# MaciejKozarzewski/AlphaGomoku

Measured on AMD Instinct MI355X. Metric: MCTS simulations/sec (self-play, 15x15 freestyle), higher is better.
Workload: dtype f16 (network, fp32 accumulate) + int/fp32 (tree)

## Files before the change

alphagomoku_amd/csrc/dev_mcts.hpp:

```cpp
#ifndef AGX_DEV_MCTS_HPP_
#define AGX_DEV_MCTS_HPP_

#include "dev_solver.hpp"
#include "root_noise.hpp"
#include "symmetry.hpp"

namespace agx
{
	namespace dev
	{
		__device__ __forceinline__ DNode* nodes_of(const EngineDev &E, int g, int arena) { return E.nodes + E.games[g].node_off[arena]; }
		__device__ __forceinline__ DEdge* edges_of(const EngineDev &E, int g, int arena) { return E.edges + E.games[g].edge_off[arena]; }
		__device__ __forceinline__ int* ht_of(const EngineDev &E, int g) { return E.ht + E.games[g].ht_off; }
		__device__ __forceinline__ void use_game_arenas(EngineDev &E, int g)
		{
			E.node_cap = E.games[g].node_cap;
			E.edge_cap = E.games[g].edge_cap;
			E.ht_cap = E.games[g].ht_cap;
		}

		__device__ inline int cache_seek(const EngineDev &E, const DNode *nodes, const int *ht, u64 hash, const u64 *cboard, int sign, int lane)
		{
			const int mask = E.ht_cap - 1;
			int slot = static_cast<int>(hash & static_cast<u64>(mask));
			for (int probes = 0; probes < E.ht_cap; probes++)
			{
				const int idx = ht[slot];
				if (idx == 0)
					return -1;
				const DNode &nd = nodes[idx - 1];
				bool same = (nd.hash == hash) && (nd.sign_to_move == sign);
				if (same)
				{
					const bool word_ok = (lane < BWORDS) ? (nd.cboard[lane] == cboard[lane]) : true;
					same = (__ballot(!word_ok) == 0);
				}
				if (same)
					return idx - 1;
				slot = (slot + 1) & mask;
			}
			return -1;
		}
		__device__ __forceinline__ void node_head(DNode &dst, const DNode &src)
		{
			dst.edge_begin = src.edge_begin;
			dst.win = src.win;
			dst.draw = src.draw;
			dst.moves_left = src.moves_left;
			dst.visits = src.visits;
			dst.score = src.score;
			dst.n_edges = src.n_edges;
			dst.depth = src.depth;
			dst.vl = src.vl;
			dst.sign_to_move = src.sign_to_move;
			dst.flags = src.flags;
			dst.hash = src.hash;
		}
		__device__ inline int cache_seek_head(const EngineDev &E, const DNode *nodes, const int *ht, u64 hash, const u64 *cboard, int sign, int lane, DNode &head)
		{
			const int mask = E.ht_cap - 1;
			int slot = static_cast<int>(hash & static_cast<u64>(mask));
			for (int probes = 0; probes < E.ht_cap; probes++)
			{
				const int idx = ht[slot];
				if (idx == 0)
					return -1;
				const DNode &nd = nodes[idx - 1];
				DNode h;
				node_head(h, nd);
				const u64 word = (lane < BWORDS) ? nd.cboard[lane] : 0ull;
				bool same = (h.hash == hash) && (h.sign_to_move == sign);
				if (same)
				{
					const bool word_ok = (lane < BWORDS) ? (word == cboard[lane]) : true;
					same = (__ballot(!word_ok) == 0);
				}
				if (same)
				{
					head = h;
					return idx - 1;
				}
				slot = (slot + 1) & mask;
			}
			return -1;
		}
		__device__ inline void cache_insert(const EngineDev &E, int *ht, u64 hash, int node)
		{
			const int mask = E.ht_cap - 1;
			int slot = static_cast<int>(hash & static_cast<u64>(mask));
			while (ht[slot] != 0)
				slot = (slot + 1) & mask;
			ht[slot] = node + 1;
		}

		__device__ inline bool has_leak(const EngineDev &E, const DEdge &e, bool node_found, uint32_t node_score, float node_win, float node_draw)
		{
			if (!node_found || E.leak_threshold >= 1.0f)
				return false;
			if (e.score != s_invert_up(node_score))
				return true;
			const float inv_win = 1.0f - (node_win + node_draw);
			const float dw = e.win - inv_win, dd = e.draw - node_draw;
			return (fabsf(dw) + fabsf(dd)) > E.leak_threshold;
		}

		__device__ __forceinline__ unsigned long long symmetry_mix(unsigned long long z)
		{
			z += 0x9E3779B97F4A7C15ull;
			z = (z ^ (z >> 30)) * 0xBF58476D1CE4E5B9ull;
			z = (z ^ (z >> 27)) * 0x94D049BB133111EBull;
			return z ^ (z >> 31);
		}

		__device__ __forceinline__ void wave_argmax(float &value, int &index)
		{
			const uint32_t bits = __float_as_uint(value);
			const uint32_t key = (bits & 0x80000000u) ? ~bits : (bits | 0x80000000u);
			const uint32_t best = wave_reduce_umax(key);
			const uint32_t mine = (key == best) ? (0x7FFFFFFFu - static_cast<uint32_t>(index)) : 0u;
			index = static_cast<int>(0x7FFFFFFFu - wave_reduce_umax(mine));
			value = __uint_as_float((best & 0x80000000u) ? (best & 0x7FFFFFFFu) : ~best);
		}
		__device__ __forceinline__ uint32_t wave_max_u32(uint32_t v)
		{
			return wave_reduce_umax(v);
		}

		__device__ inline int select_edge(const EngineDev &E, const DNode &nd, const DEdge *edges, int lane, unsigned long long &edge_reads, const float *noisy_priors)
		{
			const int total = nd.visits + nd.vl;
			float c_puct = E.c_puct;
			if (E.c_scale != 0.0f)
				c_puct = static_cast<float>(static_cast<double>(E.c_puct) + static_cast<double>(E.c_scale) * det_log(static_cast<double>(total)));
			const float parent_sqrt_visit = static_cast<float>(static_cast<double>(c_puct) * sqrt(static_cast<double>(total)));
			float initial_q = 0.0f;
			if (E.init_to == 1)
				initial_q = nd.win + 0.5f * nd.draw;
			else if (E.init_to == 2)
				initial_q = 0.5f;

			float best_value = -3.402823466e+38f;
			int best = 0x7FFFFFFF;
			for (int i = lane; i < nd.n_edges; i += 64)
			{
				const DEdge e = edges[nd.edge_begin + i];
				float value;
				switch (s_pv(e.score))
				{
					case 0:
						value = -1000.0f + s_distance(e.score);
						break;
					case 1:
						value = 0.5f;
						break;
					case 3:
						value = +1000.0f - s_distance(e.score);
						break;
					default:
					{
						const int vl = e.flag_vl & 0x7FFF;
						const bool being_expanded = (e.flag_vl & 0x8000u) != 0;
						const float visits = 1.0e-8f + e.visits;
						const float virtual_loss = static_cast<float>(vl);
						const float vl_factor = visits / (visits + virtual_loss);
						const float expectation = e.win + 0.5f * e.draw;
						float Q;
						if (E.init_to == 0)
							Q = being_expanded ? -1000.0f : expectation * vl_factor;
						else
						{
							Q = initial_q;
							if (being_expanded)
								Q = -1000.0f;
							else if (e.visits > 0)
								Q = expectation * vl_factor;
						}
						const float prior = (noisy_priors != nullptr) ? noisy_priors[i] : e.prior;
						const float U = prior * parent_sqrt_visit / (1.0f + e.visits + vl);
						value = Q + U;
						break;
					}
				}
				if (value > best_value)
				{
					best_value = value;
					best = i;
				}
			}
			edge_reads += nd.n_edges;
			wave_argmax(best_value, best);
			return nd.edge_begin + best;
		}

		__device__ inline void correct_information_leak(DNode *nodes, DEdge *edges, const DTask &t, int path_len, int final_node, int lane)
		{
			float child_win = nodes[final_node].win, child_draw = nodes[final_node].draw;
			uint32_t child_score = nodes[final_node].score;
			for (int i = path_len - 1; i >= 0; i--)
			{
				const int node = t.path_node[i], e = t.path_edge[i];
				DNode nd;
				node_head(nd, nodes[node]);
				DEdge ed = edges[e];
				const float cw = ed.win, cd = ed.draw;
				const float tw = 1.0f - (child_win + child_draw), td = child_draw;
				const float scale = static_cast<float>(ed.visits) / static_cast<float>(nd.visits);
				const float nw = nd.win + (tw - cw) * scale, ndr = nd.draw + (td - cd) * scale;
				ed.win = tw;
				ed.draw = td;
				nd.win = nw;
				nd.draw = ndr;
				const uint32_t new_score = s_invert_up(child_score);
				ed.score = static_cast<uint16_t>(new_score);
				uint32_t result = 0;
				for (int j = lane; j < nd.n_edges; j += 64)
					result = max(result, (nd.edge_begin + j == e) ? new_score : static_cast<uint32_t>(edges[nd.edge_begin + j].score));
				result = wave_max_u32(result);
				if (((nd.flags & 4) != 0) || s_win(result) || s_unproven(result))
					nd.score = static_cast<uint16_t>(result);
				if (lane == 0)
				{
					nodes[node].win = nd.win;
					nodes[node].draw = nd.draw;
					nodes[node].score = nd.score;
					edges[e].win = ed.win;
					edges[e].draw = ed.draw;
					edges[e].score = ed.score;
				}
				child_win = nd.win;
				child_draw = nd.draw;
				child_score = nd.score;
			}
		}
		__device__ inline void cancel_virtual_loss(DNode *nodes, DEdge *edges, const DTask &t, int path_len, int lane)
		{
			for (int i = lane; i < path_len; i += 64)
			{
				nodes[t.path_node[i]].vl--;
				DEdge &e = edges[t.path_edge[i]];
				e.flag_vl = static_cast<uint16_t>((e.flag_vl & 0x8000u) | (((e.flag_vl & 0x7FFF) - 1) & 0x7FFF));
			}
		}

		__device__ inline u64 full_hash(const EngineDev &E, const uint8_t *board, int sign, int lane)
		{
			u64 h = 0;
			for (int i = lane; i < E.hw; i += 64)
				h ^= E.nc_keys[3 + 3 * i + board[i]];
			return wave_reduce_xor64(h) ^ E.nc_keys[sign];
		}
	}
}

#endif
```

alphagomoku_amd/csrc/engine.hip:

```cpp
#include "agx_internal.hpp"
#include "engine_types.hpp"
#include "dev_mcts.hpp"
#include "tables_host.hpp"
#include "renju_static.hpp"
#include "root_noise.hpp"
#include "sample_v201.hpp"

#include <vector>
#include <thread>
#include <chrono>
#include <mutex>
#include <cstring>
#include <algorithm>

using namespace agx;
using namespace agx::dev;

namespace
{
	__device__ __forceinline__ void select_batch(EngineDev &E, int tg, int g, int lane, uint8_t *sh_board, u64 *sh_cboard, const u64 *sh_keys)
	{
		GameState &gs = E.games[tg];
		GameState &ls = E.games[g];
		DNode *nodes = nodes_of(E, tg, gs.arena);
		DEdge *edges = edges_of(E, tg, gs.arena);
		const int *ht = ht_of(E, tg);
		const int n = E.n;

		int n_tasks = ls.n_tasks;
		int trials = 2 * E.batch_limit;
		unsigned long long st_levels = 0, st_edges = 0, st_leaks = 0, st_proven = 0, st_dup = 0;
		while (n_tasks < E.batch_limit)
		{
			const int root = gs.root;
			const int sims = (root < 0) ? 0 : nodes[root].visits;
			if (sims > E.max_sims)
				break;
			if (E.noise_type != 0 && root >= 0 && !gs.noise_ready && nodes[root].n_edges > 0)
			{
				if (lane == 0)
				{
					const DNode rn = nodes[root];
					const DEdge *root_edges = edges + rn.edge_begin;
					make_root_noise(E.noise_type, E.noise_weight, E.noise_seed, gs.opening_id, gs.n_moves, rn.n_edges, [&](int i) { return root_edges[i].prior; },
							E.noise + static_cast<size_t>(tg) * E.hw);
					gs.noise_ready = 1;
				}
				__threadfence_block();
				__syncthreads();
			}
			DTask &t = E.tasks[static_cast<size_t>(g) * E.batch + n_tasks];
			n_tasks++;
			for (int i = lane; i < E.hw; i += 64)
				sh_board[i] = gs.board[i];
			if (lane < BWORDS)
				sh_cboard[lane] = gs.cboard[lane];
			__syncthreads();
			int path_len = 0, final_node = -1, out = 0, sign = gs.sign_to_move;
			u64 hash = gs.root_hash;
			int last_edge = -1;
			int node = root;
			DNode nd;
			if (node >= 0)
				node_head(nd, nodes[node]);
			while (node >= 0)
			{
				if (path_len >= PATH_CAP)
				{
					if (lane == 0)
						ls.error = ERR_PATH_CAPACITY;
					break;
				}
				const int e = select_edge(E, nd, edges, lane, st_edges, (node == root && gs.noise_ready) ? E.noise + static_cast<size_t>(tg) * E.hw : nullptr);
				st_levels++;
				const DEdge ee = edges[e];
				const uint32_t mv = ee.move;
				const int s = mv & 3, cell = ((mv >> 2) & 127) * n + ((mv >> 9) & 127);
				const uint16_t flag_vl = static_cast<uint16_t>((ee.flag_vl & 0x8000u) | (((ee.flag_vl & 0x7FFF) + 1) & 0x7FFF));
				if (lane == 0)
				{
					sh_board[cell] = static_cast<uint8_t>(s);
					sh_cboard[cell >> 5] |= static_cast<u64>(s) << (2 * (cell & 31));
					t.path_node[path_len] = node;
					t.path_edge[path_len] = e;
					nodes[node].vl = static_cast<int16_t>(nd.vl + 1);
					edges[e].flag_vl = flag_vl;
				}
				hash ^= sh_keys[3 + 3 * cell] ^ sh_keys[3 + 3 * cell + s] ^ sh_keys[sign] ^ sh_keys[3 - s];
				sign = 3 - s;
				path_len++;
				last_edge = e;
				__syncthreads();
				if (s_proven(ee.score))
				{
					out = 2;
					break;
				}
				DNode child;
				node = cache_seek_head(E, nodes, ht, hash, sh_cboard, sign, lane, child);
				final_node = node;
				if (node < 0 && lane == 0)
					edges[e].flag_vl = static_cast<uint16_t>(flag_vl | 0x8000u);
				if (has_leak(E, ee, node >= 0, child.score, child.win, child.draw))
				{
					out = 1;
					break;
				}
				nd = child;
			}
			for (int i = lane; i < E.hw; i += 64)
				t.board[i] = sh_board[i];
			if (lane < BWORDS)
				t.cboard[lane] = sh_cboard[lane];
			if (lane == 0)
			{
				t.path_len = path_len;
				t.final_node = final_node;
				t.n_edges = 0;
				t.flags = t.flags & (TF_STATICALLY_SOLVED | TF_RECURSIVELY_SOLVED);
				t.sign_to_move = sign;
				t.score = s_unknown(0);
				t.win = 0.0f;
				t.draw = 0.0f;
				t.needs_nn = 0;
				t.hash = hash;
				if (out == 0 && path_len > gs.max_depth)
					gs.max_depth = path_len;
			}
			__syncthreads();
			if (path_len == 0)
				break;
			for (int i = 0; i < n_tasks - 1; i++)
			{
				const DTask &o = E.tasks[static_cast<size_t>(g) * E.batch + i];
				if (o.path_len > 0 && o.path_edge[o.path_len - 1] == last_edge)
				{
					st_dup++;
					break;
				}
			}
			if (out == 1)
			{
				correct_information_leak(nodes, edges, t, path_len, final_node, lane);
				cancel_virtual_loss(nodes, edges, t, path_len, lane);
				st_leaks++;
				n_tasks--;
			}
			if (out == 2 && lane == 0)
			{
				const uint32_t sc = edges[last_edge].score;
				float w, d;
				s_to_value(sc, w, d);
				t.final_node = -1;
				t.sign_to_move = 3 - sign;
				t.score = sc;
				t.win = w;
				t.draw = d;
				t.flags |= TF_BY_SOLVER | TF_SKIP_EDGE_GENERATION;
			}
			if (out == 2)
				st_proven++;
			__syncthreads();
			if (--trials <= 0)
				break;
		}
		if (lane == 0)
		{
			ls.n_tasks = n_tasks;
			ls.stats[2] += st_leaks;
			ls.stats[3] += st_proven;
			ls.stats[6] += st_levels;
			ls.stats[7] += st_edges;
			ls.stats[9] += st_dup;
		}
	}
	__global__ __launch_bounds__(64) void k_select(EngineDev E)
	{
		__shared__ uint8_t sh_board[MAXHW];
		__shared__ u64 sh_cboard[BWORDS];
		__shared__ u64 sh_keys[3 * (1 + MAXHW)];
		const int g = E.g0 + blockIdx.x, lane = threadIdx.x;
		const int tg = E.shared_tree ? 0 : g;
		GameState &gs = E.games[tg];
		if (!gs.active || gs.error != 0 || gs.outcome != 0 || gs.grow_pending)
			return;
		use_game_arenas(E, tg);
		for (int i = lane; i < 3 * (1 + E.hw); i += 64)
			sh_keys[i] = E.nc_keys[i];
		if (!E.shared_tree)
		{
			if (!gs.solve_pending)
				select_batch(E, g, g, lane, sh_board, sh_cboard, sh_keys);
			return;
		}
		for (int t = E.grp_first; t < E.grp_first + E.grp_count; t++)
		{
			if (E.games[t].error == 0)
				select_batch(E, 0, t, lane, sh_board, sh_cboard, sh_keys);
			__syncthreads();
		}
	}

	constexpr float SPEC_PARK_FRACTION = 0.90f;
	struct ParkCtl
	{
			int count;
			int threshold;
	};
	template<class SH>
	__device__ __forceinline__ void park_copy_tails(const SH &sh, const EngineDev &E, int from, int to, int lane)
	{
		lane = fresh_lane(lane);
// ... 1113 lines not shown
						const int src = (r < K) ? (0xFFFF - static_cast<int>(sort_keys[r] & 0xFFFFu)) : 0;
						g_mv[c] = e_move[src];
						g_sc[c] = e_score[src];
						g_p[c] = e_prior[src];
						g_w[c] = e_win[src];
						g_d[c] = e_draw[src];
						kept += __popcll(__ballot(r < K && g_p[c] >= threshold));
					}
					__syncthreads();
#pragma unroll
					for (int c = 0; c < 7; c++)
					{
						const int r = c * 64 + lane;
						if (r < kept)
						{
							e_move[r] = g_mv[c];
							e_score[r] = g_sc[c];
							e_prior[r] = g_p[c];
							e_win[r] = g_w[c];
							e_draw[r] = g_d[c];
						}
					}
					__syncthreads();
					n_e = kept;
				}
				float sum = 0.0f;
				for (int base = 0; base < n_e; base += 64)
				{
					const int mine_i = __float_as_int((base + lane < n_e) ? e_prior[base + lane] : 0.0f);
					const int m = min(64, n_e - base);
					int j = 0;
					for (; j + 4 <= m; j += 4)
					{
						sum += __int_as_float(__builtin_amdgcn_readlane(mine_i, j));
						sum += __int_as_float(__builtin_amdgcn_readlane(mine_i, j + 1));
						sum += __int_as_float(__builtin_amdgcn_readlane(mine_i, j + 2));
						sum += __int_as_float(__builtin_amdgcn_readlane(mine_i, j + 3));
					}
					for (; j < m; j++)
						sum += __int_as_float(__builtin_amdgcn_readlane(mine_i, j));
				}
				if (sum == 0.0f)
				{
					const float u = 1.0f / n_e;
					for (int i = lane; i < n_e; i += 64)
						e_prior[i] = u;
				}
				else
				{
					const float inv = 1.0f / sum;
					for (int i = lane; i < n_e; i += 64)
						e_prior[i] = e_prior[i] * inv;
				}
				__syncthreads();
			}
			else
				n_e = 0;

			int final_node = t.final_node;
			if (n_e > 0)
			{
				const int found = cache_seek(E, nodes, ht, t.hash, t.cboard, sign, lane);
				if (found < 0)
				{
					const int nid = gs.n_nodes, ebeg = gs.n_edges;
					if (nid >= E.node_cap || ebeg + n_e > E.edge_cap || 2 * (nid + 1) > E.ht_cap)
					{
						if (lane == 0)
							gs.error = (nid >= E.node_cap) ? ERR_NODE_CAPACITY : ((ebeg + n_e > E.edge_cap) ? ERR_EDGE_CAPACITY : ERR_HASH_TABLE);
						__syncthreads();
						return;
					}
					uint32_t max_score = 0;
					for (int i = lane; i < n_e; i += 64)
					{
						DEdge e;
						e.prior = e_prior[i];
						e.win = e_win[i];
						e.draw = e_draw[i];
						e.visits = 0;
						e.move = e_move[i];
						e.score = e_score[i];
						e.flag_vl = 0;
						e.pad = 0;
						edges[ebeg + i] = e;
						max_score = max(max_score, static_cast<uint32_t>(e_score[i]));
					}
					max_score = wave_max_u32(max_score);
					if (lane < BWORDS)
						nodes[nid].cboard[lane] = t.cboard[lane];
					if (lane == 0)
					{
						DNode &nd = nodes[nid];
						nd.edge_begin = ebeg;
						nd.n_edges = static_cast<int16_t>(n_e);
						nd.depth = static_cast<int16_t>(gs.n_moves + path_len);
						nd.vl = 0;
						nd.sign_to_move = static_cast<uint8_t>(sign);
						nd.pad8 = 0;
						nd.hash = t.hash;
						nd.visits = 1;
						const float tmp = static_cast<float>(1.0 / 1);
						float w = 0.0f + (win - 0.0f) * tmp, d = 0.0f + (draw - 0.0f) * tmp;
						nd.win = fmaxf(0.0f, fminf(1.0f, w));
						nd.draw = fmaxf(0.0f, fminf(1.0f, d));
						nd.moves_left = 0.0f + (moves_left - 0.0f) / 1;
						uint16_t nf = 0;
						if ((flags & TF_MUST_DEFEND) || (n_e + nd.depth) == hw)
							nf |= 4;
						nf |= ((flags & TF_STATICALLY_SOLVED) ? 8 : 0) | ((flags & TF_RECURSIVELY_SOLVED) ? 16 : 0) | ((flags & TF_MUST_DEFEND) ? 32 : 0);
						if (path_len == 0)
							nf |= 2;
						nd.flags = nf;
						nd.score = static_cast<uint16_t>(s_unknown(0));
						if ((nf & 4) || s_win(max_score) || s_unproven(max_score))
							nd.score = static_cast<uint16_t>(max_score);
						cache_insert(E, ht, t.hash, nid);
						gs.n_nodes = nid + 1;
						gs.n_edges = ebeg + n_e;
						if (path_len == 0)
							gs.root = nid;
					}
					final_node = nid;
					__syncthreads();
				}
				else
				{
					final_node = found;
					wasted++;
					if (path_len > 0)
					{
						const DEdge le = edges[t.path_edge[path_len - 1]];
						if (has_leak(E, le, true, nodes[found].score, nodes[found].win, nodes[found].draw))
							correct_information_leak(nodes, edges, t, path_len, final_node, lane);
					}
				}
			}

			if (lane == 0)
			{
				t.final_node = final_node;
				t.win = win;
				t.draw = draw;
				t.moves_left = moves_left;
				t.flags = flags;
			}
			__syncthreads();
		}

		for (int k = 0; k < n_tasks; k++)
		{
			DTask &t = E.tasks[static_cast<size_t>(g) * E.batch + k];
			const float win = t.win, draw = t.draw;
			const int path_len = t.path_len, sign = t.sign_to_move, final_node = t.final_node;
			float ml = t.moves_left;
			bool have_child = final_node >= 0;
			uint32_t child_score = have_child ? nodes[final_node].score : 0u;
#if AGX_WIDE_BACKUP
			if (path_len <= 64)
			{
				const bool mine = lane < path_len;
				const int node = mine ? t.path_node[lane] : 0, e = mine ? t.path_edge[lane] : 0;
				DNode nd;
				node_head(nd, nodes[node]);
				DEdge ed = edges[e];
				float ml_i = ml;
				for (int k = path_len - 1; k > lane; k--)
					ml_i += 1.0f;
				float vw = win, vd = draw;
				if (nd.sign_to_move != sign)
				{
					vw = 1.0f - (win + draw);
					vd = draw;
				}
				nd.visits++;
				const float tn = static_cast<float>(1.0 / nd.visits);
				nd.win = fmaxf(0.0f, fminf(1.0f, nd.win + (vw - nd.win) * tn));
				nd.draw = fmaxf(0.0f, fminf(1.0f, nd.draw + (vd - nd.draw) * tn));
				ed.visits++;
				const float te = 1.0f / ed.visits;
				ed.win = fmaxf(0.0f, fminf(1.0f, ed.win + (vw - ed.win) * te));
				ed.draw = fmaxf(0.0f, fminf(1.0f, ed.draw + (vd - ed.draw) * te));
				nd.moves_left += (ml_i - nd.moves_left) / nd.visits;
				nd.vl--;
				ed.flag_vl = static_cast<uint16_t>(((ed.flag_vl & 0x7FFF) - 1) & 0x7FFF);
				uint32_t others = 0;
				constexpr int LEVELS = 8, LOADS = (MAXHW + 63) / 64;
				for (int base = 0; base < path_len; base += LEVELS)
				{
					uint32_t sc[LEVELS][LOADS];
#pragma unroll
					for (int u = 0; u < LEVELS; u++)
					{
						const int lv = min(base + u, path_len - 1);
						const int eb = __builtin_amdgcn_readlane(nd.edge_begin, __builtin_amdgcn_readfirstlane(lv));
						const int ne = __builtin_amdgcn_readlane(static_cast<int>(nd.n_edges), __builtin_amdgcn_readfirstlane(lv));
						const int ee = __builtin_amdgcn_readlane(e, __builtin_amdgcn_readfirstlane(lv));
#pragma unroll
						for (int jj = 0; jj < LOADS; jj++)
						{
							const int j = lane + 64 * jj;
							sc[u][jj] = (base + u < path_len && j < ne && eb + j != ee) ? static_cast<uint32_t>(edges[eb + j].score) : 0u;
						}
					}
#pragma unroll
					for (int u = 0; u < LEVELS; u++)
					{
						uint32_t m = 0;
#pragma unroll
						for (int jj = 0; jj < LOADS; jj++)
							m = max(m, sc[u][jj]);
						m = wave_max_u32(m);
						if (lane == base + u)
							others = m;
					}
// ... 183 lines not shown
		for (int i = tid; i < E.hw; i += 256)
			h ^= E.nc_keys[3 + 3 * i + gs.board[i]];
		block_reduce_xor(h, scratch, tid);
		if (tid == 0)
			gs.root_hash = h ^ E.nc_keys[gs.sign_to_move];
		__syncthreads();
	}

	template<int TPB, bool DropRoot = false>
	__device__ void rebase_tree(const EngineDev &E0, int t, int tid, u64 *scratch, int *scan_nodes, int *scan_edges)
	{
		EngineDev E = E0;
		use_game_arenas(E, t);
		GameState &gs = E.games[t];
		const int lane = tid & 63, wave = tid >> 6;
		DNode *nodes = nodes_of(E, t, gs.arena);
		DEdge *edges = edges_of(E, t, gs.arena);
		DNode *dst_nodes = nodes_of(E, t, gs.arena ^ 1);
		DEdge *dst_edges = edges_of(E, t, gs.arena ^ 1);
		int *ht = ht_of(E, t);
		for (int i = tid; i < E.ht_cap; i += TPB)
			ht[i] = 0;
		const int total = gs.n_nodes;
		int node_base = 0, edge_base = 0;
		u64 drop_hash = 0;
		if constexpr (DropRoot)
		{
			for (int i = tid; i < E.hw; i += TPB)
				drop_hash ^= E.nc_keys[3 + 3 * i + gs.board[i]];
			block_reduce_xor<TPB>(drop_hash, scratch, tid);
			drop_hash ^= E.nc_keys[gs.sign_to_move];
		}
		__syncthreads();
		for (int base = 0; base < total; base += TPB)
		{
			const int i = base + tid;
			int keep = 0, ne = 0;
			if (i < total)
			{
				keep = 1;
				u64 differs = 0;
				for (int w = 0; w < BWORDS; w++)
				{
					const u64 from = gs.cboard[w], to = nodes[i].cboard[w];
					if (((from ^ to) & from) != 0)
						keep = 0;
					differs |= from ^ to;
				}
				if constexpr (DropRoot)
				{
					if (differs == 0 && nodes[i].hash == drop_hash && nodes[i].sign_to_move == gs.sign_to_move)
						keep = 0;
				}
				ne = keep ? nodes[i].n_edges : 0;
			}
			scan_nodes[tid] = keep;
			scan_edges[tid] = ne;
			__syncthreads();
			for (int o = 1; o < TPB; o <<= 1)
			{
				const int a = (tid >= o) ? scan_nodes[tid - o] : 0, b = (tid >= o) ? scan_edges[tid - o] : 0;
				__syncthreads();
				scan_nodes[tid] += a;
				scan_edges[tid] += b;
				__syncthreads();
			}
			int cp_src = 0, cp_dst = 0;
			if (keep)
			{
				const int ni = node_base + scan_nodes[tid] - 1, eb = edge_base + scan_edges[tid] - ne;
				DNode nd = nodes[i];
				cp_src = nd.edge_begin;
				cp_dst = eb;
				nd.edge_begin = eb;
				dst_nodes[ni] = nd;
				const int mask = E.ht_cap - 1;
				int slot = static_cast<int>(nd.hash & static_cast<u64>(mask));
				while (atomicCAS(&ht[slot], 0, ni + 1) != 0)
					slot = (slot + 1) & mask;
			}
			{
				const u64 *src64 = reinterpret_cast<const u64*>(edges);
				u64 *dst64 = reinterpret_cast<u64*>(dst_edges);
				for (int k = 0; k < 64; k++)
				{
					const int words = 3 * __builtin_amdgcn_readlane(ne, k);
					if (words == 0)
						continue;
					const size_t so = 3 * static_cast<size_t>(__builtin_amdgcn_readlane(cp_src, k)), dof = 3 * static_cast<size_t>(__builtin_amdgcn_readlane(cp_dst, k));
					for (int d = lane; d < words; d += 256)
					{
						const u64 w0 = src64[so + d];
						const u64 w1 = (d + 64 < words) ? src64[so + d + 64] : 0ull;
						const u64 w2 = (d + 128 < words) ? src64[so + d + 128] : 0ull;
						const u64 w3 = (d + 192 < words) ? src64[so + d + 192] : 0ull;
						dst64[dof + d] = w0;
						if (d + 64 < words)
							dst64[dof + d + 64] = w1;
						if (d + 128 < words)
							dst64[dof + d + 128] = w2;
						if (d + 192 < words)
							dst64[dof + d + 192] = w3;
					}
				}
			}
			node_base += scan_nodes[TPB - 1];
			edge_base += scan_edges[TPB - 1];
			__syncthreads();
		}
		u64 h = 0;
		for (int i = tid; i < E.hw; i += TPB)
			h ^= E.nc_keys[3 + 3 * i + gs.board[i]];
		block_reduce_xor<TPB>(h, scratch, tid);
		if (tid == 0)
		{
			gs.root_hash = h ^ E.nc_keys[gs.sign_to_move];
			gs.n_nodes = node_base;
			gs.n_edges = edge_base;
			gs.arena ^= 1;
			gs.generation = (gs.generation + 1) % 64;
			gs.max_depth = 0;
		}
		__syncthreads();
		if (wave == 0)
		{
			const int found = cache_seek(E, dst_nodes, ht, gs.root_hash, gs.cboard, gs.sign_to_move, lane);
			if (lane == 0)
			{
				gs.root = found;
				if (found >= 0)
					dst_nodes[found].flags |= 2;
			}
		}
		__syncthreads();
	}

	__global__ __launch_bounds__(256) void k_begin(EngineDev E)
	{
		__shared__ u64 scratch[4];
		const int g = blockIdx.x, tid = threadIdx.x;
		GameState &gs = E.games[g];
		__shared__ int sh_id;
		if (tid == 0)
		{
			sh_id = E.shared_tree ? 0 : g;
			gs.generation = 0;
			gs.error = 0;
			gs.games_done = 0;
			gs.arena = 0;
			for (int i = 0; i < 12; i++)
				gs.stats[i] = 0;
		}
		__syncthreads();
		if (E.match_mode)
		{
			clear_tree_and_table(E, g, tid);
			if (tid == 0)
			{
				gs.active = 0;
				gs.root = -1;
				gs.n_nodes = 0;
				gs.n_edges = 0;
				gs.n_tasks = 0;
				gs.need_move = 0;
				gs.solve_pos = 0;
				gs.solve_pending = 0;
				park_forget_game(E, g);
				gs.outcome = 0;
				gs.n_moves = 0;
				gs.restart_id = (g < E.n_games / 2) ? -1 : 0;
				gs.match_score[0] = gs.match_score[1] = gs.match_score[2] = gs.match_score[3] = 0;
			}
		}
		else if (sh_id < E.n_openings)
			begin_game(E, g, sh_id, tid, scratch);
		else if (tid == 0)
		{
			gs.active = 0;
			gs.restart_id = -1;
		}
	}

	constexpr int ADV_THREADS = 1024;
	__global__ __launch_bounds__(ADV_THREADS) void k_advance(EngineDev E)
	{
// ... 1887 lines not shown
	cfg->game_end_capacity = 0;
	cfg->speculative_solver = 0;
	cfg->speculative_waves = 0;
	cfg->force_expand_root = 1;
	cfg->search_buffers = 0;
	cfg->noise_type = 0;
	cfg->noise_weight = 0.0f;
	cfg->noise_seed = 0x2545F4914F6CDD1Dull;
	return AGX_OK;
}

#if defined(AGX_QUICK) && !defined(AGX_QUICK_RENJU)
#define AGX_QUICK_RENJU false
#endif
typedef void (*SpecKernel)(EngineDev, int);
static SpecKernel spec_kernel(int rules, int n)
{
#ifdef AGX_QUICK
	(void) rules;
	(void) n;
	return k_search_spec<AGX_QUICK_RENJU, 15>;
#else
	if (rules == AGX_RENJU)
		return (n == 15) ? k_search_spec<true, 15> : k_search_spec<true, 0>;
	if (n == 15)
		return k_search_spec<false, 15>;
	return (n == 20) ? k_search_spec<false, 20> : k_search_spec<false, 0>;
#endif
}
static int spec_resident_waves_per_cu(int rules, int n)
{
	int blocks = 0;
	if (hipOccupancyMaxActiveBlocksPerMultiprocessor(&blocks, reinterpret_cast<const void*>(spec_kernel(rules, n)), 64, 0) != hipSuccess || blocks <= 0)
	{
		(void) hipGetLastError();
		return 12;
	}
	return blocks;
}
static int engine_create(const AgxEngineConfig *cfg, AgxEngine **out, int sizing_cus)
{
	AGX_REQUIRE(cfg != nullptr && out != nullptr, AGX_ERR_INVALID, "agx_engine_create: null argument");
	AGX_REQUIRE(cfg->rules >= 0 && cfg->rules <= AGX_CARO6, AGX_ERR_INVALID, "agx_engine_create: unknown rules %d", cfg->rules);
	AGX_REQUIRE(cfg->board_size >= 5 && cfg->board_size <= MAXN, AGX_ERR_UNSUPPORTED, "agx_engine_create: board size %d not in [5, %d]", cfg->board_size, MAXN);
	AGX_REQUIRE(cfg->n_games > 0 && cfg->max_batch_size > 0 && cfg->max_simulations > 0, AGX_ERR_INVALID, "agx_engine_create: non-positive sizes");
	AGX_REQUIRE(cfg->tss_max_positions >= 1 && cfg->tss_max_positions <= 1000, AGX_ERR_UNSUPPORTED, "agx_engine_create: tss_max_positions must be in [1, 1000]");
	AGX_REQUIRE(cfg->init_to >= 0 && cfg->init_to <= 3, AGX_ERR_INVALID, "agx_engine_create: init_to must be 0..3");
	AGX_REQUIRE(cfg->solver_yield_fraction >= 0.0f && cfg->solver_yield_fraction <= 1.0f, AGX_ERR_INVALID, "agx_engine_create: solver_yield_fraction must be in [0, 1]");
	AGX_REQUIRE(cfg->final_selector >= 0 && cfg->final_selector <= 5, AGX_ERR_INVALID, "agx_engine_create: final_selector must be 0..5");
	AGX_REQUIRE(cfg->noise_type >= 0 && cfg->noise_type <= 3, AGX_ERR_INVALID, "agx_engine_create: noise_type must be 0 (none), 1 (custom), 2 (dirichlet) or 3 (gumbel)");
	AGX_REQUIRE(cfg->policy_temperature >= 0.0f, AGX_ERR_INVALID, "agx_engine_create: policy_temperature must not be negative");
	AGX_REQUIRE(!cfg->match_mode || cfg->n_games % 2 == 0, AGX_ERR_INVALID, "agx_engine_create: match_mode pairs the trees, n_games must be even");
	AGX_REQUIRE(cfg->noise_weight >= 0.0f && cfg->noise_weight <= 1.0f, AGX_ERR_INVALID, "agx_engine_create: noise_weight must be in [0, 1]");
	AGX_REQUIRE(cfg->search_buffers >= 0 && cfg->search_buffers <= 2, AGX_ERR_INVALID, "agx_engine_create: search_buffers must be 0, 1 or 2");
	{
		const int threads = std::max(1, cfg->search_threads), buffers = (cfg->search_buffers == 2) ? 2 : 1;
		AGX_REQUIRE((threads == 1 && buffers == 1) || (threads * buffers == cfg->n_games && !cfg->match_mode && cfg->solver_yield_fraction == 0.0f), AGX_ERR_INVALID,
				"agx_engine_create: search_threads > 1 / search_buffers = 2 make the pool ONE tree searched by n_games task buffers: n_games must equal "
				"search_threads x buffers (%d x %d), no match_mode, no yielding", threads, buffers);
	}
	AGX_REQUIRE(cfg->record_format >= 0 && cfg->record_format <= 3, AGX_ERR_INVALID, "agx_engine_create: record_format must be 0..3 (bit 0 edge snapshots, bit 1 format-201 samples)");

	AgxEngine *e = new AgxEngine();
	e->cfg = *cfg;
	e->sizing_only = sizing_cus > 0;
	e->sizing_cus = sizing_cus;
	if (const char *fuse = std::getenv("AGX_FUSE_SELECT"))
		e->fuse_select = std::atoi(fuse) != 0;
	EngineDev &d = e->dev;
	std::memset(&d, 0, sizeof(d));
	d.rules = cfg->rules;
	d.n = cfg->board_size;
	d.hw = d.n * d.n;
	d.draw_after = (cfg->draw_after > 0) ? cfg->draw_after : d.hw;
	d.n_games = cfg->n_games;
	d.batch = cfg->max_batch_size;
	d.max_sims = cfg->max_simulations;
	d.c_puct = cfg->exploration_constant;
	d.c_scale = cfg->exploration_scaling;
	d.init_to = cfg->init_to;
	d.leak_threshold = cfg->information_leak_threshold;
	d.expansion_threshold = cfg->policy_expansion_threshold;
	d.max_children = (cfg->max_children > 0) ? cfg->max_children : 0x7FFFFFFF;
	d.tss_max_nodes = cfg->tss_max_positions;
	d.tss_max_depth = 100;
	d.solve_time_ticks = 0ull;
	d.batch_limit = d.batch;
	d.yield_fraction = cfg->solver_yield_fraction;
	d.final_selector = cfg->final_selector;
	d.use_symmetries = cfg->use_symmetries;
	d.symmetry_seed = cfg->symmetry_seed;
	d.noise_type = (cfg->noise_weight > 0.0f) ? cfg->noise_type : 0;
	d.noise_weight = cfg->noise_weight;
	d.noise_seed = cfg->noise_seed;
	const size_t buckets = round_pow2(std::max<size_t>(cfg->tss_table_entries, 4)) / 4;
	d.tt_bucket_mask = buckets - 1;
	d.zobrist_seed = cfg->zobrist_seed;
	d.node_cap = cfg->node_capacity > 0 ? cfg->node_capacity : 8192;
	d.edge_cap = cfg->edge_capacity > 0 ? cfg->edge_capacity : 524288;
	d.edge_cap += d.edge_cap & 1;
	d.ht_cap = static_cast<int>(round_pow2(4 * static_cast<size_t>(d.node_cap)));
	d.act_cap = d.hw * (d.hw + 1) / 2 + 64;
	d.record_cap = cfg->record_capacity > 0 ? cfg->record_capacity : d.n_games * d.hw;
	d.record_edge_cap = cfg->record_edge_capacity > 0 ? cfg->record_edge_capacity : d.record_cap * 64;
	d.record_format = cfg->record_format;
	d.sample_cap = cfg->record_sample_capacity > 0 ? cfg->record_sample_capacity
			: static_cast<int>(std::min<size_t>(static_cast<size_t>(d.record_cap) * (16 + 6 * static_cast<size_t>(d.hw) + 2), 0x7FFFFFF0u));
	d.game_end_cap = cfg->game_end_capacity > 0 ? cfg->game_end_capacity : std::max(2 * d.n_games, d.record_cap / 16);

	HostTables tables;
	build_host_tables(cfg->rules, tables);
	std::vector<uint64_t> nc_keys(3 + 3 * d.hw);
	uint64_t st = cfg->zobrist_seed ^ 0x5851F42D4C957F2Dull;
	for (auto &k : nc_keys)
		k = splitmix64(st);
	e->zobrist.resize(4 * d.hw);
	st = cfg->zobrist_seed;
	for (auto &k : e->zobrist)
		k = splitmix64(st);

	int status = AGX_OK;
	const size_t G = d.n_games;
#define AGX_TRY(expr) if (status == AGX_OK) status = (expr)
	AGX_TRY(dev_alloc(e, &d.games, G));
	const double reserve = (cfg->arena_reserve >= 0.0f) ? cfg->arena_reserve : 1.0;
	const size_t node_total = static_cast<size_t>(static_cast<double>(G * 2 * d.node_cap) * (1.0 + reserve));
	const size_t edge_total = static_cast<size_t>(static_cast<double>(G * 2 * d.edge_cap) * (1.0 + reserve));
	const size_t ht_total = static_cast<size_t>(static_cast<double>(G * d.ht_cap) * (1.0 + reserve));
	AGX_TRY(dev_alloc(e, &d.nodes, node_total));
	AGX_TRY(dev_alloc(e, &d.edges, edge_total));
	AGX_TRY(dev_alloc(e, &d.ht, ht_total));
	AGX_TRY(dev_alloc(e, &d.heap, 1));
	AGX_TRY(dev_alloc(e, &d.free_bundles, static_cast<size_t>(ARENA_CLASSES) * G));
	AGX_TRY(dev_alloc(e, &d.tasks, G * d.batch));
	e->speculative = cfg->speculative_solver != 0 && cfg->tss_max_positions <= 250 && cfg->max_batch_size <= 16;
	if (e->speculative)
	{
		int cus = e->sizing_cus, device_of_engine = 0;
		if (!e->sizing_only)
		{
			(void) hipGetDevice(&device_of_engine);
			(void) hipDeviceGetAttribute(&cus, hipDeviceAttributeMultiprocessorCount, device_of_engine);
		}
		const int per_cu = spec_resident_waves_per_cu(cfg->rules, cfg->board_size);
		e->spec_waves = (cfg->speculative_waves > 0) ? cfg->speculative_waves : std::min<long long>(static_cast<long long>(per_cu) * std::max(1, cus), std::max<long long>(64, static_cast<long long>(G) * cfg->max_batch_size));
		e->spec_waves = std::min(e->spec_waves, SPEC_QUEUE_SLACK);
	}
	const bool parking = e->speculative && cfg->rules == AGX_RENJU && cfg->solver_yield_fraction > 0.0f && !cfg->match_mode && std::max(1, cfg->search_threads) == 1;
	const size_t areas = G + static_cast<size_t>(std::max(e->spec_waves, 16)) + (parking ? SPEC_PARK_POOL : 0);
	d.park_area0 = static_cast<int>(G) + std::max(e->spec_waves, 16);
	d.spec_on = e->speculative ? 1 : 0;
	d.park_fraction = parking ? SPEC_PARK_FRACTION : 0.0f;
	if (const char *pf = std::getenv("AGX_PARK_FRACTION"))
		if (parking && std::atof(pf) > 0.0)
			d.park_fraction = std::min(1.0f, static_cast<float>(std::atof(pf)));
	AGX_TRY(dev_alloc(e, &d.park_slot, G * d.batch));
	AGX_TRY(dev_alloc(e, &d.park_owner, SPEC_PARK_POOL));
	AGX_TRY(dev_alloc(e, &d.parts_done, 2 * G));
	if (!e->sizing_only)
		(void) hipMemset(d.parts_done, 0, 2 * G * sizeof(int));
	AGX_TRY(dev_alloc(e, &d.park_lds, parking ? static_cast<size_t>(SPEC_PARK_POOL) * SPEC_PARK_WORDS : 1));
	if (!e->sizing_only)
		(void) hipMemset(d.park_slot, 0, G * d.batch * sizeof(int));
	if (!e->sizing_only)
		(void) hipMemset(d.park_owner, 0, SPEC_PARK_POOL * sizeof(int));
	AGX_TRY(dev_alloc(e, &d.act, areas * d.act_cap));
// ... 2190 lines not shown
```

alphagomoku_amd/csrc/engine_types.hpp:

```cpp
#ifndef AGX_ENGINE_TYPES_HPP_
#define AGX_ENGINE_TYPES_HPP_

#include <cstdint>

namespace agx
{
	constexpr int MAXN = 20;
	constexpr int MAXHW = MAXN * MAXN;
	constexpr int BWORDS = 13;
	constexpr int PATH_CAP = 256;
	constexpr int SPEC_PARK_POOL = 128;
	constexpr int SPEC_PARK_WORDS = 2048 + 8;
	constexpr int MAX_FRAMES = 104;
	constexpr int OPENING_CAP = 32;

	struct alignas(16) FrameBytes { uint32_t w[8]; };

	struct DEdge
	{
			float prior;
			float win;
			float draw;
			int32_t visits;
			uint16_t move;
			uint16_t score;
			uint16_t flag_vl;
			uint16_t pad;
	};
	static_assert(sizeof(DEdge) == 24, "edge record must stay 24 bytes");

	struct DNode
	{
			int32_t edge_begin;
			float win;
			float draw;
			float moves_left;
			int32_t visits;
			uint16_t score;
			int16_t n_edges;
			int16_t depth;
			int16_t vl;
			uint8_t sign_to_move;
			uint8_t pad8;
			uint16_t flags;
			uint64_t hash;
			uint64_t cboard[BWORDS];
	};
	static_assert(sizeof(DNode) == 144, "node record layout");

	enum TaskFlags : uint32_t
	{
		TF_MUST_DEFEND = 1, TF_BY_NETWORK = 2, TF_BY_SOLVER = 4, TF_SKIP_EDGE_GENERATION = 8, TF_STATICALLY_SOLVED = 16, TF_RECURSIVELY_SOLVED = 32
	};

	struct DTask
	{
			int32_t path_len;
			int32_t final_node;
			int32_t n_edges;
			uint32_t flags;
			int32_t sign_to_move;
			uint32_t score;
			float win;
			float draw;
			float moves_left;
			int32_t needs_nn;
			int32_t symmetry;
			int32_t pad;
			uint64_t hash;
			uint64_t cboard[BWORDS];
			int32_t path_node[PATH_CAP];
			int32_t path_edge[PATH_CAP];
			uint8_t board[MAXHW];
			uint16_t emove[MAXHW];
			uint16_t escore[MAXHW];
	};

	struct GameState
	{
			int32_t active;
			int32_t sign_to_move;
			int32_t n_moves;
			int32_t outcome;
			int32_t root;
			int32_t n_nodes;
			int32_t n_edges;
			int32_t arena;
			int32_t n_tasks;
			int32_t need_move;
			int32_t generation;
			int32_t error;
			int32_t opening_id;
			int32_t games_done;
			int32_t solve_pos;
			int32_t solve_pending;
			int32_t nn_queued;
			int32_t noise_ready;
			int32_t my_sign;
			int32_t restart_id;
			int32_t match_score[4];
			int32_t arena_class;
			int32_t grow_pending;
			int32_t node_cap, edge_cap, ht_cap, grow_count;
			int32_t grow_owner, max_depth;
			uint64_t node_off[2], edge_off[2], ht_off;
			uint64_t new_node_off[2], new_edge_off[2], new_ht_off;
			uint64_t root_hash;
			uint64_t cboard[BWORDS];
			unsigned long long prof[8];
			unsigned long long dprof[24];
			unsigned long long spec_stats[4];
			unsigned long long stats[12];
			uint8_t board[MAXHW];
			uint16_t moves[MAXHW];
	};

	struct MoveRecordHeader
	{
			int32_t game_serial;
			int32_t move_number;
			uint16_t move;
			uint16_t root_score;
			int32_t root_visits;
			float root_win;
			float root_draw;
			int32_t n_edges;
			int32_t edge_offset;
			int32_t root_flags;
			int32_t game_slot;
			int32_t game_index;
			int32_t sample_offset;
			int32_t sample_bytes;
			int32_t outcome;
	};
	struct GameEndRecord
	{
			int32_t game_serial, game_slot, game_index;
			int32_t outcome;
			int32_t n_moves;
			uint16_t moves[MAXHW];
	};

	constexpr int SPEC_OV_CAP = 256;
	constexpr int SPEC_COUNTER0 = 64;
	constexpr int SPEC_QUEUE_SLACK = 8192;
	constexpr int N_COUNTERS = 192;
	struct SpecTask
	{
			int32_t solved;
			int32_t count;
			int32_t overflow;
			int32_t nodes;
			uint32_t flags0;
			float moves_left0;
			uint32_t pad[2];
			uint32_t dirty[SPEC_OV_CAP / 32];
			uint32_t keys[SPEC_OV_CAP];
	};

	constexpr int ARENA_CLASSES = 6;

	struct ArenaBundle
	{
			uint64_t node_off[2], edge_off[2], ht_off;
	};
	struct ArenaHeap
	{
			uint64_t node_cursor, edge_cursor, ht_cursor;
			uint64_t node_total, edge_total, ht_total;
			int32_t free_count[ARENA_CLASSES];
			int32_t free_capacity;
			int32_t grows, releases, failures, lock;
	};

	enum EngineError : int32_t
	{
		ERR_NONE = 0, ERR_NODE_CAPACITY = 1, ERR_EDGE_CAPACITY = 2, ERR_PATH_CAPACITY = 3, ERR_ACTION_STACK = 4, ERR_HASH_TABLE = 5, ERR_RECORDS = 6, ERR_FRAMES = 7, ERR_SPEC_STATE = 8,
		ERR_OVERLAY = 100
	};

	struct EngineDev
	{
			int rules, n, hw, draw_after;
			int n_games, batch, max_sims;
			int batch_limit;
			float c_puct, c_scale;
			int init_to;
			float leak_threshold, expansion_threshold;
			int max_children;
			float policy_temperature;
			int tss_max_nodes, tss_max_depth;
			unsigned long long solve_time_ticks;
			unsigned long long zobrist_seed;
			unsigned long long tt_bucket_mask;
			int node_cap, edge_cap, ht_cap, act_cap;
			int record_cap, record_edge_cap;
			int record_format;
			int sample_cap;
			int game_end_cap;
			int n_openings;
			float yield_fraction;
			int yield_counter;
			int final_selector, use_symmetries;
			unsigned long long symmetry_seed;
			int noise_type;
			float noise_weight;
			unsigned long long noise_seed;
			float *noise;
			int g0;
			int nn_counter;
			GameState *games;
			DNode *nodes;
			DEdge *edges;
			int *ht;
			ArenaHeap *heap;
			ArenaBundle *free_bundles;
			DTask *tasks;
			uint32_t *act;
			uint16_t *list_spill;
			FrameBytes *frame_spill;
			uint64_t *snap_spill;
			uint64_t *tt;
			const uint8_t *t_pattern;
			const uint8_t *t_ho3;
			const uint8_t *t_threat;
			const uint8_t *t_threat_packed;
			const uint16_t *t_defense;
			const uint64_t *nc_keys;
			const uint64_t *zob;
			const uint16_t *openings;
			uint32_t *nn_features;
			float *nn_policy;
			float *nn_value;
			float *nn_q;
			int has_q;
			int match_merged;
			int prune_root;
			int match_mode;
			int shared_tree;
			int search_buffers;
			int tt_mod;
			int grp_first, grp_count;
			int spec_on;
			int spec_group;
			int *spec_watchdog;
			unsigned long long *spec_trace;
			unsigned long long *spec_prof;
			int spec_waves;
			int *spec_items;
			int *spec_left;
			SpecTask *spec_tasks;
			uint64_t *spec_overlay;
			int *park_slot;
			int *park_owner;
			int *parts_done;
			uint64_t *park_lds;
			int park_area0;
			float park_fraction;
			int *nn_list;
			int *counters;
			MoveRecordHeader *records;
			DEdge *record_edges;
			uint8_t *samples;
			GameEndRecord *game_ends;
	};
}

#endif
```

include/agx.h:

```cpp
#ifndef AGX_H_
#define AGX_H_

#include <stddef.h>
#include <stdint.h>

#ifdef __cplusplus
extern "C" {
#endif

#define AGX_OK 0
#define AGX_ERR_INVALID 1
#define AGX_ERR_HIP 2
#define AGX_ERR_UNSUPPORTED 3
#define AGX_ERR_STATE 4

enum AgxRules { AGX_FREESTYLE = 0, AGX_STANDARD = 1, AGX_RENJU = 2, AGX_CARO5 = 3, AGX_CARO6 = 4 };

enum AgxSign { AGX_NONE = 0, AGX_CROSS = 1, AGX_CIRCLE = 2, AGX_ILLEGAL = 3 };

const char* agx_last_error(void);
int agx_version(void);
const char* agx_build_hash(void);
int agx_set_device(int device);
int agx_device_count(int* count);
// ... 10 lines not shown
	int action_values;
} AgxNetDesc;

typedef struct AgxNet AgxNet;

size_t agx_net_blob_floats(const AgxNetDesc* desc);
int agx_net_create(const AgxNetDesc* desc, AgxNet** out);
int agx_net_load_weights(AgxNet* net, const float* h_blob, size_t n_floats);
int agx_nn_forward(AgxNet* net, const uint32_t* d_features, int batch, float* d_policy, float* d_value, void* stream);
int agx_nn_forward_pvq(AgxNet* net, const uint32_t* d_features, int batch, float* d_policy, float* d_value, float* d_action_values, void* stream);
int agx_net_description(const AgxNet* net, AgxNetDesc* out);
int agx_net_set_launch_width(AgxNet* net, int workgroups);
int agx_net_destroy(AgxNet* net);

int agx_nn_forward_indirect(AgxNet* net, const uint32_t* d_features, const int* d_slot_list, const int* d_count, int max_batch,
		float* d_policy, float* d_value, void* stream);
int agx_nn_forward_indirect_pvq(AgxNet* net, const uint32_t* d_features, const int* d_slot_list, const int* d_count, int max_batch,
		float* d_policy, float* d_value, float* d_action_values, void* stream);

enum AgxNetArchitecture { AGX_ARCH_RESNET = 0, AGX_ARCH_CONVNEXT = 1, AGX_ARCH_BOTTLENECK = 2 };
size_t agx_net_blob_floats_ex(const AgxNetDesc* desc, int architecture, int moves_left);
int agx_net_create_ex(const AgxNetDesc* desc, int architecture, int moves_left, AgxNet** out);
int agx_net_architecture(const AgxNet* net, int* architecture, int* moves_left);
int agx_nn_forward_pvqm(AgxNet* net, const uint32_t* d_features, int batch, float* d_policy, float* d_value, float* d_action_values,
		float* d_moves_left, void* stream);
int agx_nn_forward_indirect_pvqm(AgxNet* net, const uint32_t* d_features, const int* d_slot_list, const int* d_count, int max_batch,
		float* d_policy, float* d_value, float* d_action_values, float* d_moves_left, void* stream);

typedef struct AgxEngineConfig
{
	int rules;
	int board_size;
	int draw_after;
	int n_games;
	int max_batch_size;
	int max_simulations;
	float exploration_constant;
	float exploration_scaling;
	int init_to;
	float information_leak_threshold;
	float policy_expansion_threshold;
	int tss_max_positions;
	uint64_t tss_table_entries;
	uint64_t zobrist_seed;
	int node_capacity;
	int edge_capacity;
	int record_capacity;
	int record_edge_capacity;
	float solver_yield_fraction;
	int final_selector;
	int use_symmetries;
	uint64_t symmetry_seed;
	int max_children;
	int noise_type;
	float noise_weight;
	uint64_t noise_seed;
	int action_values;
	int match_mode;
	float policy_temperature;
	float arena_reserve;
	int search_threads;
	int record_format;
	int record_sample_capacity;
	int game_end_capacity;
	int speculative_solver;
	int speculative_waves;
	int force_expand_root;
	int search_buffers;
} AgxEngineConfig;

typedef struct AgxEngine AgxEngine;

typedef struct AgxEngineBuffers
{
	uint32_t* d_nn_features;
	float* d_nn_policy;
	float* d_nn_value;
	float* d_nn_action_values;
	int* d_nn_list;
	int* d_nn_count;
	int slots;
	int cells;
} AgxEngineBuffers;

typedef struct AgxEngineStats
{
	unsigned long long evaluated_nodes;
	unsigned long long network_evaluations;
	unsigned long long information_leaks;
	unsigned long long proven_edge_visits;
	unsigned long long wasted_expansions;
	unsigned long long duplicate_selections;
	unsigned long long solver_nodes;
	unsigned long long select_levels;
	unsigned long long select_edge_reads;
	unsigned long long moves_played;
	unsigned long long peak_nodes;
	unsigned long long peak_edges;
	int games_finished;
	int openings_taken;
	int active_games;
	int records_used;
	int record_edges_used;
	int first_error;
	int arena_grows;
	int arena_releases;
	int arena_failures;
	int arena_max_class;
	float arena_heap_used;
	int speculative_parks;
	unsigned long long speculative_solves;
	unsigned long long speculative_reruns;
	unsigned long long speculative_deferrals;
} AgxEngineStats;

typedef struct AgxEdgeView
{
	float prior, win, draw;
	int32_t visits;
	uint16_t move;
	uint16_t score;
	uint16_t flag_and_virtual_loss;
	uint16_t reserved;
} AgxEdgeView;

typedef struct AgxGameInfo
{
	int active, sign_to_move, n_moves, outcome, error, opening_id, games_done, n_nodes, n_edges;
	int root_visits;
	float root_win, root_draw;
	int root_score;
	int root_edges;
	int grow_pending;
	int arena_class;
	float root_moves_left;
	int max_depth;
} AgxGameInfo;

typedef struct AgxMoveRecord
{
	int game_serial, move_number;
	uint16_t move, root_score;
	int root_visits;
	float root_win, root_draw;
	int n_edges, edge_offset;
	int root_flags;
	int game_slot;
	int game_index;
	int sample_offset;
	int sample_bytes;
	int outcome;
} AgxMoveRecord;

typedef struct AgxGameEnd
{
	int game_serial, game_slot, game_index;
	int outcome;
	int n_moves;
	uint16_t moves[400];
} AgxGameEnd;

typedef struct AgxSavedGame
{
	int game_slot, game_index;
	int opening_id, sign_to_move, nn_queued, n_moves;
	uint16_t moves[400];
// ... 360 lines not shown
```

Measured before the change: 1.035 million.

## Cache child node links in edge padding to skip hash-table probes during selection

Reuses the spare 16-bit pad field of each edge as a direct link to the child node index, filled on expansion, cache hit and first lookup. Selection then checks the linked node's hash and sign instead of probing the hash table and comparing the full board. It also broadcasts the chosen edge from the owning lane with readlane instead of re-reading it from memory. Links are cleared when the tree is rebased. The fast path is limited to nodes below 65535, and a mismatched link aborts with a new error code, which is a correctness risk.

```diff
diff --git a/alphagomoku_amd/csrc/dev_mcts.hpp b/alphagomoku_amd/csrc/dev_mcts.hpp
--- a/alphagomoku_amd/csrc/dev_mcts.hpp
+++ b/alphagomoku_amd/csrc/dev_mcts.hpp
@@ -84,6 +84,13 @@
 			}
 			return -1;
 		}
+		__device__ __forceinline__ int linked_seek_head(const DNode *nodes, int n_nodes, uint32_t child, u64 hash, int sign, DNode &head)
+		{
+			if (static_cast<int>(child) > n_nodes)
+				return -2;
+			node_head(head, nodes[child - 1]);
+			return (head.hash == hash && head.sign_to_move == sign) ? static_cast<int>(child) - 1 : -2;
+		}
 		__device__ inline void cache_insert(const EngineDev &E, int *ht, u64 hash, int node)
 		{
 			const int mask = E.ht_cap - 1;
@@ -126,7 +133,8 @@
 			return wave_reduce_umax(v);
 		}
 
-		__device__ inline int select_edge(const EngineDev &E, const DNode &nd, const DEdge *edges, int lane, unsigned long long &edge_reads, const float *noisy_priors)
+		__device__ inline int select_edge(const EngineDev &E, const DNode &nd, const DEdge *edges, int lane, unsigned long long &edge_reads, const float *noisy_priors,
+				DEdge &chosen)
 		{
 			const int total = nd.visits + nd.vl;
 			float c_puct = E.c_puct;
@@ -141,6 +149,7 @@
 
 			float best_value = -3.402823466e+38f;
 			int best = 0x7FFFFFFF;
+			DEdge mine = { };
 			for (int i = lane; i < nd.n_edges; i += 64)
 			{
 				const DEdge e = edges[nd.edge_begin + i];
@@ -185,10 +194,22 @@
 				{
 					best_value = value;
 					best = i;
+					mine = e;
 				}
 			}
 			edge_reads += nd.n_edges;
 			wave_argmax(best_value, best);
+			const int owner = __builtin_amdgcn_readfirstlane(best & 63);
+			chosen.prior = __int_as_float(__builtin_amdgcn_readlane(__float_as_int(mine.prior), owner));
+			chosen.win = __int_as_float(__builtin_amdgcn_readlane(__float_as_int(mine.win), owner));
+			chosen.draw = __int_as_float(__builtin_amdgcn_readlane(__float_as_int(mine.draw), owner));
+			chosen.visits = __builtin_amdgcn_readlane(mine.visits, owner);
+			const uint32_t move_score = static_cast<uint32_t>(__builtin_amdgcn_readlane(static_cast<int>(mine.move | (static_cast<uint32_t>(mine.score) << 16)), owner));
+			const uint32_t vl_child = static_cast<uint32_t>(__builtin_amdgcn_readlane(static_cast<int>(mine.flag_vl | (static_cast<uint32_t>(mine.child) << 16)), owner));
+			chosen.move = static_cast<uint16_t>(move_score);
+			chosen.score = static_cast<uint16_t>(move_score >> 16);
+			chosen.flag_vl = static_cast<uint16_t>(vl_child);
+			chosen.child = static_cast<uint16_t>(vl_child >> 16);
 			return nd.edge_begin + best;
 		}
 
diff --git a/alphagomoku_amd/csrc/engine.hip b/alphagomoku_amd/csrc/engine.hip
--- a/alphagomoku_amd/csrc/engine.hip
+++ b/alphagomoku_amd/csrc/engine.hip
@@ -30,6 +30,8 @@
 		int n_tasks = ls.n_tasks;
 		int trials = 2 * E.batch_limit;
 		unsigned long long st_levels = 0, st_edges = 0, st_leaks = 0, st_proven = 0, st_dup = 0;
+		const int n_nodes = gs.n_nodes;
+		bool stale_link = false;
 		while (n_tasks < E.batch_limit)
 		{
 			const int root = gs.root;
@@ -71,9 +73,9 @@
 						ls.error = ERR_PATH_CAPACITY;
 					break;
 				}
-				const int e = select_edge(E, nd, edges, lane, st_edges, (node == root && gs.noise_ready) ? E.noise + static_cast<size_t>(tg) * E.hw : nullptr);
+				DEdge ee;
+				const int e = select_edge(E, nd, edges, lane, st_edges, (node == root && gs.noise_ready) ? E.noise + static_cast<size_t>(tg) * E.hw : nullptr, ee);
 				st_levels++;
-				const DEdge ee = edges[e];
 				const uint32_t mv = ee.move;
 				const int s = mv & 3, cell = ((mv >> 2) & 127) * n + ((mv >> 9) & 127);
 				const uint16_t flag_vl = static_cast<uint16_t>((ee.flag_vl & 0x8000u) | (((ee.flag_vl & 0x7FFF) + 1) & 0x7FFF));
@@ -97,7 +99,25 @@
 					break;
 				}
 				DNode child;
-				node = cache_seek_head(E, nodes, ht, hash, sh_cboard, sign, lane, child);
+				const uint32_t link = (E.link_max > 0) ? ee.child : 0u;
+				if (link != 0)
+				{
+					node = linked_seek_head(nodes, n_nodes, link, hash, sign, child);
+					if (node < -1)
+					{
+						if (lane == 0)
+							ls.error = ERR_STALE_CHILD_LINK;
+						stale_link = true;
+						final_node = -1;
+						break;
+					}
+				}
+				else
+				{
+					node = cache_seek_head(E, nodes, ht, hash, sh_cboard, sign, lane, child);
+					if (node >= 0 && node < E.link_max && lane == 0)
+						edges[e].child = static_cast<uint16_t>(node + 1);
+				}
 				final_node = node;
 				if (node < 0 && lane == 0)
 					edges[e].flag_vl = static_cast<uint16_t>(flag_vl | 0x8000u);
@@ -128,6 +148,8 @@
 					gs.max_depth = path_len;
 			}
 			__syncthreads();
+			if (stale_link)
+				break;
 			if (path_len == 0)
 				break;
 			for (int i = 0; i < n_tasks - 1; i++)
@@ -1407,7 +1429,7 @@
 						e.move = e_move[i];
 						e.score = e_score[i];
 						e.flag_vl = 0;
-						e.pad = 0;
+						e.child = 0;
 						edges[ebeg + i] = e;
 						max_score = max(max_score, static_cast<uint32_t>(e_score[i]));
 					}
@@ -1445,6 +1467,8 @@
 						gs.n_edges = ebeg + n_e;
 						if (path_len == 0)
 							gs.root = nid;
+						else if (nid < E.link_max)
+							edges[t.path_edge[path_len - 1]].child = static_cast<uint16_t>(nid + 1);
 					}
 					final_node = nid;
 					__syncthreads();
@@ -1456,6 +1480,8 @@
 					if (path_len > 0)
 					{
 						const DEdge le = edges[t.path_edge[path_len - 1]];
+						if (found < E.link_max && lane == 0)
+							edges[t.path_edge[path_len - 1]].child = static_cast<uint16_t>(found + 1);
 						if (has_leak(E, le, true, nodes[found].score, nodes[found].win, nodes[found].draw))
 							correct_information_leak(nodes, edges, t, path_len, final_node, lane);
 					}
@@ -1805,25 +1831,33 @@
 			{
 				const u64 *src64 = reinterpret_cast<const u64*>(edges);
 				u64 *dst64 = reinterpret_cast<u64*>(dst_edges);
+				constexpr u64 NO_LINK = 0x0000FFFFFFFFFFFFull;
+				const int lane3 = lane % 3;
+				const u64 mask_first[3] = { (lane3 == 2) ? NO_LINK : ~0ull, (lane3 == 1) ? NO_LINK : ~0ull, (lane3 == 0) ? NO_LINK : ~0ull };
 				for (int k = 0; k < 64; k++)
 				{
 					const int words = 3 * __builtin_amdgcn_readlane(ne, k);
 					if (words == 0)
 						continue;
 					const size_t so = 3 * static_cast<size_t>(__builtin_amdgcn_readlane(cp_src, k)), dof = 3 * static_cast<size_t>(__builtin_amdgcn_readlane(cp_dst, k));
+					u64 m0 = mask_first[0], m1 = mask_first[1], m2 = mask_first[2];
 					for (int d = lane; d < words; d += 256)
 					{
 						const u64 w0 = src64[so + d];
 						const u64 w1 = (d + 64 < words) ? src64[so + d + 64] : 0ull;
 						const u64 w2 = (d + 128 < words) ? src64[so + d + 128] : 0ull;
 						const u64 w3 = (d + 192 < words) ? src64[so + d + 192] : 0ull;
-						dst64[dof + d] = w0;
+						dst64[dof + d] = w0 & m0;
 						if (d + 64 < words)
-							dst64[dof + d + 64] = w1;
+							dst64[dof + d + 64] = w1 & m1;
 						if (d + 128 < words)
-							dst64[dof + d + 128] = w2;
+							dst64[dof + d + 128] = w2 & m2;
 						if (d + 192 < words)
-							dst64[dof + d + 192] = w3;
+							dst64[dof + d + 192] = w3 & m0;
+						const u64 m = m0;
+						m0 = m1;
+						m1 = m2;
+						m2 = m;
 					}
 				}
 			}
@@ -3877,6 +3911,12 @@
 	d.leak_threshold = cfg->information_leak_threshold;
 	d.expansion_threshold = cfg->policy_expansion_threshold;
 	d.max_children = (cfg->max_children > 0) ? cfg->max_children : 0x7FFFFFFF;
+	d.link_max = CHILD_LINK_LIMIT;
+	if (const char *limit = std::getenv("AGX_CHILD_LINK_MAX"))
+		d.link_max = std::min(std::max(std::atoi(limit), 0), CHILD_LINK_LIMIT);
+	if (const char *links = std::getenv("AGX_CHILD_LINKS"))
+		if (std::atoi(links) == 0)
+			d.link_max = 0;
 	d.tss_max_nodes = cfg->tss_max_positions;
 	d.tss_max_depth = 100;
 	d.solve_time_ticks = 0ull;
diff --git a/alphagomoku_amd/csrc/engine_types.hpp b/alphagomoku_amd/csrc/engine_types.hpp
--- a/alphagomoku_amd/csrc/engine_types.hpp
+++ b/alphagomoku_amd/csrc/engine_types.hpp
@@ -1,6 +1,7 @@
 #ifndef AGX_ENGINE_TYPES_HPP_
 #define AGX_ENGINE_TYPES_HPP_
 
+#include <cstddef>
 #include <cstdint>
 
 namespace agx
@@ -25,9 +26,11 @@
 			uint16_t move;
 			uint16_t score;
 			uint16_t flag_vl;
-			uint16_t pad;
+			uint16_t child;
 	};
 	static_assert(sizeof(DEdge) == 24, "edge record must stay 24 bytes");
+	static_assert(offsetof(DEdge, child) == 22, "rebase_tree clears the link as the top 16 bits of a record's third 8-byte word");
+	constexpr int CHILD_LINK_LIMIT = 65535;
 
 	struct DNode
 	{
@@ -176,6 +179,7 @@
 	enum EngineError : int32_t
 	{
 		ERR_NONE = 0, ERR_NODE_CAPACITY = 1, ERR_EDGE_CAPACITY = 2, ERR_PATH_CAPACITY = 3, ERR_ACTION_STACK = 4, ERR_HASH_TABLE = 5, ERR_RECORDS = 6, ERR_FRAMES = 7, ERR_SPEC_STATE = 8,
+		ERR_STALE_CHILD_LINK = 9,
 		ERR_OVERLAY = 100
 	};
 
@@ -188,6 +192,7 @@
 			int init_to;
 			float leak_threshold, expansion_threshold;
 			int max_children;
+			int link_max;
 			float policy_temperature;
 			int tss_max_nodes, tss_max_depth;
 			unsigned long long solve_time_ticks;
diff --git a/include/agx.h b/include/agx.h
--- a/include/agx.h
+++ b/include/agx.h
@@ -116,6 +116,8 @@
 	int slots;
 	int cells;
 } AgxEngineBuffers;
+
+enum { AGX_ENGINE_ERROR_STALE_CHILD_LINK = 9 };
 
 typedef struct AgxEngineStats
 {
```

Result: no change. 1.039 million (median of 4 runs) (+0.4%).
